# jw007123/hp-Adaptive-Signed-Distance-Field-Octree

Measured on AMD Instinct MI355X. Metric: Query() Mpts/sec at targetError=1e-5 (union3 field, 10M SplitMix64 pts per GPU, HBM-resident); Create() ms reported as create_ms, higher is better.
Workload: dtype f64

## Files before the change

### hp-adaptive-signed-distance-field-octree_amd/__init__.py

```python
import ctypes as C
import os

import numpy as np

_HERE = os.path.dirname(os.path.abspath(__file__))
_WHICH = os.environ.get("HPSDF_LIBRARY", "")
LIB_PATH = os.path.join(_HERE, "lib", "libhpsdf_%s.so" % _WHICH if _WHICH else "libhpsdf.so")
_LIB = None

OK = 0
ERR_INVALID_ARGUMENT = 1
ERR_NO_DEVICE = 2
ERR_HIP = 3
ERR_BAD_BLOCK = 4
ERR_UNSUPPORTED = 5
ERR_STATE = 6
ERR_OUT_OF_MEMORY = 7
ERR_OPEN_MESH = 8
ERR_BUILD_LIMIT = 9
ABI_VERSION = 4
PRIM_SPHERE, PRIM_BOX, PRIM_TORUS_Y, PRIM_PLANE = 0, 1, 2, 3
OP_UNION, OP_INTERSECT, OP_SUBTRACT = 0, 1, 2
JOB_HEADER_DOUBLES = 9
DEFAULT_JOBS_PER_ROUND = 1024
# ... 56 lines not shown
CALLBACK = C.CFUNCTYPE(C.c_double, C.POINTER(C.c_double), C.c_uint64, C.c_void_p)

_SIGNATURES = {
    "hpsdf_config_default": (C.c_int, [C.POINTER(PodConfig)]),
    "hpsdf_last_error": (C.c_char_p, []),
    "hpsdf_version": (C.c_char_p, []),
    "hpsdf_tables_get": (C.c_int, [C.c_void_p] * 7),
    "hpsdf_ctx_create": (C.c_int, [C.c_int, C.c_void_p, C.POINTER(C.c_void_p)]),
    "hpsdf_ctx_destroy": (C.c_int, [C.c_void_p]),
    "hpsdf_ctx_set_stream": (C.c_int, [C.c_void_p, C.c_void_p]),
    "hpsdf_ctx_synchronize": (C.c_int, [C.c_void_p]),
    "hpsdf_ctx_set_fast_fit": (C.c_int, [C.c_void_p, C.c_int]),
    "hpsdf_ctx_set_fit_mode": (C.c_int, [C.c_void_p, C.c_int]),
    "hpsdf_ctx_get_fit_mode": (C.c_int, [C.c_void_p, C.POINTER(C.c_int)]),
    "hpsdf_ctx_set_split_min_degree": (C.c_int, [C.c_void_p, C.c_int]),
    "hpsdf_ctx_set_block_allocator": (None, [C.c_void_p] * 4),
    "hpsdf_field_release_host_copies": (C.c_int, [C.c_void_p]),
    "hpsdf_set_mesh_face_rule": (None, [C.c_int]),
    "hpsdf_get_mesh_face_rule": (C.c_int, []),
    "hpsdf_set_reduction_order": (None, [C.c_int]),
    "hpsdf_get_reduction_order": (C.c_int, []),
    "hpsdf_ctx_stream": (C.c_void_p, [C.c_void_p]),
    "hpsdf_abi_version": (C.c_int, []),
    "hpsdf_ctx_set_reduction_order": (C.c_int, [C.c_void_p, C.c_int]),
    "hpsdf_ctx_get_reduction_order": (C.c_int, [C.c_void_p, C.POINTER(C.c_int)]),
    "hpsdf_ctx_set_mesh_face_rule": (C.c_int, [C.c_void_p, C.c_int]),
    "hpsdf_ctx_get_mesh_face_rule": (C.c_int, [C.c_void_p, C.POINTER(C.c_int)]),
    "hpsdf_ctx_set_build_limits": (C.c_int, [C.c_void_p, C.c_uint64, C.c_uint64]),
    "hpsdf_ctx_get_build_limits": (C.c_int, [C.c_void_p, C.POINTER(C.c_uint64), C.POINTER(C.c_uint64)]),
    "hpsdf_field_create_analytic": (C.c_int, [C.POINTER(Prim), C.c_int, C.POINTER(C.c_void_p)]),
# ... 106 lines not shown
                                                       C.POINTER(ContinuityStats)]),
    "hpsdf_continuity_matrix": (C.c_int, [C.c_void_p, C.c_size_t, C.c_uint64, C.POINTER(C.POINTER(C.c_uint64)),
                                          C.POINTER(C.POINTER(C.c_uint64)), C.POINTER(C.POINTER(C.c_double)),
                                          C.POINTER(ContinuityStats)]),
    "hpsdf_continuity_matrix_device": (C.c_int, [C.c_void_p, C.c_void_p, C.c_size_t, C.POINTER(C.POINTER(C.c_uint64)),
                                          C.POINTER(C.POINTER(C.c_uint64)), C.POINTER(C.POINTER(C.c_double)),
                                          C.POINTER(ContinuityStats)]),
    "hpsdf_continuity_last_stats": (C.c_int, [C.POINTER(ContinuityStats)]),
    "hpsdf_create": (C.c_int, [C.c_void_p, C.POINTER(PodConfig), C.c_void_p, C.c_uint64, C.POINTER(C.c_void_p),
                               C.POINTER(C.c_size_t), C.POINTER(BuildStats)]),
    "hpsdf_create_distributed": (C.c_int, [C.c_void_p, C.POINTER(PodConfig), C.c_void_p, C.c_uint64, C.c_int, C.c_int, C.c_void_p,
                                           C.c_void_p, C.POINTER(C.c_void_p), C.POINTER(C.c_size_t), C.POINTER(BuildStats)]),
    "hpsdf_fit_cells": (C.c_int, [C.c_void_p, C.POINTER(PodConfig), C.c_void_p, C.c_int, C.c_int, C.c_uint64, C.c_void_p, C.c_void_p]),
    "hpsdf_bench_fit": (C.c_int, [C.c_void_p, C.POINTER(PodConfig), C.c_void_p, C.c_int, C.c_int, C.c_uint64, C.c_int,
                                  C.POINTER(C.c_double)]),
}


def lib():
    global _LIB
    if _LIB is None:
        if not os.path.exists(LIB_PATH):
            raise ImportError("libhpsdf.so is not built (run __graft_entry__.build() or "
                              "python hp-adaptive-signed-distance-field-octree_amd/build.py); "
                              "there is no CPU fallback for the hot path")
        try:
            import torch
        except Exception:
            pass
        L = C.CDLL(LIB_PATH)
# ... 162 lines not shown

    def build_limits(self):
        a, b = C.c_uint64(), C.c_uint64()
        check(lib().hpsdf_ctx_get_build_limits(self.handle, C.byref(a), C.byref(b)))
        return a.value, b.value

    def set_fast_fit(self, on=True):
        check(lib().hpsdf_ctx_set_fast_fit(self.handle, 1 if on else 0))

    def set_fit_mode(self, mode):
        check(lib().hpsdf_ctx_set_fit_mode(self.handle, int(mode)))

    def set_split_min_degree(self, degree):
        check(lib().hpsdf_ctx_set_split_min_degree(self.handle, int(degree)))

    def fit_mode(self):
        m = C.c_int(0)
        check(lib().hpsdf_ctx_get_fit_mode(self.handle, C.byref(m)))
        return m.value

    def synchronize(self):
        check(lib().hpsdf_ctx_synchronize(self.handle))

    def close(self):
        if self.handle:
            lib().hpsdf_ctx_destroy(self.handle)
            self.handle = C.c_void_p()

    def __del__(self):
        try:
# ... 534 lines not shown

def bench_fit(ctx, config, field, degree, depth, n_cells, repeats=5):
    pod = config.to_pod()
    ms = C.c_double()
    check(lib().hpsdf_bench_fit(ctx.handle, C.byref(pod), field.handle, degree, depth, n_cells, repeats, C.byref(ms)))
    return ms.value


def fit_cells(ctx, config, field, degree, depth, n_cells):
    pod = config.to_pod()
    nc = int(NCOEF[degree])
    coeffs, errs = np.empty((n_cells, nc)), np.empty(n_cells)
    check(lib().hpsdf_fit_cells(ctx.handle, C.byref(pod), field.handle, degree, depth, n_cells, coeffs.ctypes.data_as(C.c_void_p),
                                errs.ctypes.data_as(C.c_void_p)))
    return coeffs, errs


class Octree:

    def __init__(self, device=0, stream=None, jobs_per_round=0):
        self._device, self._stream, self.K = device, stream, jobs_per_round
        self._ctx = None
        self._tree = None
        self.block = None
        self.config = None
        self.stats = None

    @property
    def ctx(self):
        if self._ctx is None:
# ... 419 lines not shown
```

### hp-adaptive-signed-distance-field-octree_amd/build.py

```python
import os
import shutil
import subprocess
import sys

HERE = os.path.dirname(os.path.abspath(__file__))
CSRC = os.path.join(HERE, "csrc")
LIBDIR = os.path.join(HERE, "lib")
LIB = os.path.join(LIBDIR, "libhpsdf.so")
HOOKS_LIB = os.path.join(LIBDIR, "libhpsdf_hooks.so")
HOOK_SOURCES = ["frontier.hip", "capi.cpp"]
INCLUDE = os.path.normpath(os.path.join(HERE, "..", "include"))

SOURCES = ["fit_mesh.hip", "fit_analytic.hip", "fit_samples.hip", "fit.hip", "kernels.hip", "mesh_field.hip", "frontier.hip", "fit_mfma.hip", "fit_low.hip", "mesh_build.hip", "cg.hip", "continuity_asm.hip", "surface.hip", "surface_sparse.hip", "query_gradient.hip", "query_hessian.hip", "project.hip", "cast_rays.hip", "query_bounds.hip", "integrate.hip", "tables.cpp", "builder.cpp", "mesh.cpp", "obj.cpp", "continuity.cpp", "host_query.cpp", "capi.cpp"]
HEADERS = sorted(f for f in os.listdir(CSRC) if f.endswith(".hpp"))
QUERY_SOURCES = ("kernels.hip",)
MESH_SOURCES = ("mesh_field.hip", "fit_mesh.hip")
SOURCE_GROUPS = {"query": QUERY_SOURCES, "mesh": MESH_SOURCES}
PUBLIC_HEADERS = ["hpsdf.h", "hpsdf_octree.hpp"]

FLAGS = ["-O3", "-std=c++17", "-fPIC", "-ffp-contract=off", "-fno-fast-math", "--offload-arch=gfx950",
         "-fvisibility=hidden", "-Wall", "-Wno-unused-function", "-I", INCLUDE]
FLAGS += os.environ.get("HPSDF_EXTRA_FLAGS", "").split()
FILE_FLAGS = {"fit_mfma.hip": ["-mllvm", "-amdgpu-mfma-vgpr-form=1"]}


def hipcc():
    for c in (os.environ.get("HIPCC"), "/opt/rocm/bin/hipcc", shutil.which("hipcc")):
        if c and os.path.exists(c):
            return c
    raise RuntimeError("hipcc not found: the HIP extension cannot be built (there is no CPU fallback)")


def stale():
    if not os.path.exists(LIB) or not os.path.exists(HOOKS_LIB):
        return True
    t = os.path.getmtime(LIB)
    deps = [os.path.join(CSRC, s) for s in SOURCES + HEADERS] + [os.path.join(INCLUDE, h) for h in PUBLIC_HEADERS]
    deps.append(os.path.abspath(__file__))
# ... 104 lines not shown
```

### hp-adaptive-signed-distance-field-octree_amd/csrc/capi.cpp

```cpp
#include <hip/hip_runtime_api.h>

#include <atomic>
#include <limits>
#include <cfloat>
#include <chrono>
#include <cmath>
#include <cstdio>
#include <cstdlib>
#include <cstring>
#include <memory>
#include <mutex>
#include <new>
#include <string>
#include <thread>
#include <vector>

#include "builder.hpp"
#include "continuity.hpp"
#include "frontier.hpp"
#include "block.hpp"
#include "host_call.hpp"
#include "integrate.hpp"
#include "launch.hpp"
#include "ray_cast.hpp"
#include "runtime.hpp"
#include "tree_bound.hpp"

using namespace hpsdf;

namespace hpsdf {

int loadObj(const char* path, std::vector<float>& verts, std::vector<uint64_t>& tris, std::string& err);

// ... 5 lines not shown
    g_lastError = msg;
    return code;
}
int hipFail(hipError_t e, const char* what) {
    g_lastError = std::string(what) + ": " + hipGetErrorString(e);
    (void)hipGetLastError();
    return (e == hipErrorNoDevice || e == hipErrorInvalidDevice || e == hipErrorInsufficientDriver) ? HPSDF_ERR_NO_DEVICE
                                                                                                 : HPSDF_ERR_HIP;
}

const hpsdf_field* innermost(const hpsdf_field* f) {
    while (f && f->kind == kHostTreeCsg) f = f->inner;
    return f;
}

static int envLeftAssoc() {
    const char* e = std::getenv("HPSDF_REDUCTION_ORDER");
    return e && (e[0] == 'l' || e[0] == 'L' || e[0] == '1');
}
static std::atomic<int> gLeftAssoc{envLeftAssoc()};
int reductionLeftAssoc(const hpsdf_ctx* ctx) { return ctx && ctx->reductionOrder >= 0 ? ctx->reductionOrder : gLeftAssoc.load(std::memory_order_relaxed); }
void setReductionLeftAssoc(int left) { gLeftAssoc.store(left != 0, std::memory_order_relaxed); }

static int envMeshFaceRule() {
    const char* e = std::getenv("HPSDF_MESH_FACE_RULE");
    return e && (e[0] == 'r' || e[0] == 'R' || e[0] == '1');
}
static std::atomic<int> gMeshFaceReference{envMeshFaceRule()};
int meshFaceRuleReference(const hpsdf_ctx* ctx) { return ctx && ctx->meshFaceRule >= 0 ? ctx->meshFaceRule : gMeshFaceReference.load(std::memory_order_relaxed); }
void setMeshFaceRuleReference(int on) { gMeshFaceReference.store(on != 0, std::memory_order_relaxed); }
// ... 61 lines not shown
            out->mesh.slabs = f->dSlabs;
            out->mesh.leafLog2 = f->leafLog2;
            {
                const char* pc = std::getenv("HPSDF_MESH_POOL_CAP");
                out->mesh.poolCap = pc ? (uint32_t)std::strtoul(pc, nullptr, 10) : 0xFFFFFFFFu;
            }
            out->mesh.nTris = f->nTris;
            out->mesh.nNodes = f->nBvhNodes;
            out->mesh.stats = f->dStats;
            out->mesh.faceTolOfSlack = meshFaceTolOfSlack(ctx);
            break;
        default:
            return fail(HPSDF_ERR_INVALID_ARGUMENT, "unknown field kind");
    }
    out->leftAssoc = reductionLeftAssoc(ctx);
    return HPSDF_OK;
}

}

namespace {
int treeOnContext(hpsdf_ctx* ctx, const hpsdf_tree* t, TreeDev* td = nullptr) {
    if (t->device != ctx->device) return fail(HPSDF_ERR_INVALID_ARGUMENT, "tree lives on another device");
    HPSDF_HIP(hipSetDevice(ctx->device));
    if (td) *td = t->dev, td->leftAssoc = reductionLeftAssoc(ctx);
    return HPSDF_OK;
}
}

extern "C" {
// ... 39 lines not shown
    *out = nullptr;
    int n = 0;
    hipError_t e = hipGetDeviceCount(&n);
    if (e != hipSuccess || n == 0)
        return fail(HPSDF_ERR_NO_DEVICE, std::string("no HIP device: ") + (e != hipSuccess ? hipGetErrorString(e) : "count = 0"));
    if (device < 0 || device >= n) return fail(HPSDF_ERR_INVALID_ARGUMENT, "device ordinal out of range");
    HPSDF_HIP(hipSetDevice(device));
    hpsdf_ctx* c = new hpsdf_ctx();
    c->device = device;
    c->splitMinDegree = fitSplitDefaultMinDegree();
    if (const char* fm = std::getenv("HPSDF_FIT_MODE")) {
        if (!std::strcmp(fm, "exact")) c->fitMode = HPSDF_FIT_EXACT;
        else if (!std::strcmp(fm, "fast")) c->fitMode = HPSDF_FIT_FAST;
        else if (!std::strcmp(fm, "split")) c->fitMode = HPSDF_FIT_SPLIT;
    }
    if (stream) {
        c->stream = (hipStream_t)stream;
    } else {
        hipError_t se = hipStreamCreateWithFlags(&c->stream, hipStreamNonBlocking);
        if (se != hipSuccess) {
            delete c;
            return hipFail(se, "hipStreamCreate");
        }
        c->ownsStream = true;
    }
    const Tables& T = tables();
    DeviceTables* h = new DeviceTables();
    std::memset(h, 0, sizeof(*h));
    std::memcpy(h->roots, T.roots, sizeof T.roots);
    std::memcpy(h->weights, T.weights, sizeof T.weights);
// ... 42 lines not shown
        c->ownsStream = false;
    }
    c->stream = (hipStream_t)stream;
    return HPSDF_OK;
}

int hpsdf_ctx_set_fit_mode(hpsdf_ctx* c, int mode) {
    if (!c) return fail(HPSDF_ERR_INVALID_ARGUMENT, "null context");
    if (mode != HPSDF_FIT_EXACT && mode != HPSDF_FIT_SPLIT && mode != HPSDF_FIT_FAST) return fail(HPSDF_ERR_INVALID_ARGUMENT, "unknown fit mode");
    c->fitMode = mode;
    return HPSDF_OK;
}
int hpsdf_ctx_get_fit_mode(hpsdf_ctx* c, int* mode) {
    if (!c || !mode) return fail(HPSDF_ERR_INVALID_ARGUMENT, "null argument");
    *mode = c->fitMode;
    return HPSDF_OK;
}
int hpsdf_ctx_set_build_limits(hpsdf_ctx* c, uint64_t max_nodes, uint64_t max_bytes) {
    if (!c) return fail(HPSDF_ERR_INVALID_ARGUMENT, "null context");
    c->limitNodes = max_nodes, c->limitBytes = max_bytes;
    return HPSDF_OK;
}
int hpsdf_ctx_get_build_limits(const hpsdf_ctx* c, uint64_t* max_nodes, uint64_t* max_bytes) {
    if (!c) return fail(HPSDF_ERR_INVALID_ARGUMENT, "null context");
    if (max_nodes) *max_nodes = c->limitNodes;
    if (max_bytes) *max_bytes = c->limitBytes;
    return HPSDF_OK;
}
int hpsdf_ctx_set_split_min_degree(hpsdf_ctx* c, int degree) {
    if (!c) return fail(HPSDF_ERR_INVALID_ARGUMENT, "null context");
// ... 1508 lines not shown
    if (!ctx) return fail(HPSDF_ERR_NO_DEVICE, "a device context is required");
    if (!block || !rowPtr || !col || !val) return fail(HPSDF_ERR_INVALID_ARGUMENT, "null argument");
    std::string err;
    const int rc = continuityMatrixDevice(ctx, block, size, rowPtr, col, val, stats, err);
    if (rc) return fail(rc, err);
    return HPSDF_OK;
    HPSDF_CATCH
}

int hpsdf_continuity_last_stats(hpsdf_continuity_stats* out) {
    if (!out) return fail(HPSDF_ERR_INVALID_ARGUMENT, "null out");
    *out = g_lastContinuity;
    return HPSDF_OK;
}

static int benchFit(hpsdf_ctx* ctx, const hpsdf_config* cfg, const hpsdf_field* field, int degree, int depth, uint64_t nCells, int repeats,
                    double* msPerLaunch, double* coeffsOut, double* errsOut);
int hpsdf_bench_fit(hpsdf_ctx* ctx, const hpsdf_config* cfg, const hpsdf_field* field, int degree, int depth,
                    uint64_t nCells, int repeats, double* msPerLaunch) {
    HPSDF_TRY
    if (!msPerLaunch) return fail(HPSDF_ERR_INVALID_ARGUMENT, "bad bench arguments");
    return benchFit(ctx, cfg, field, degree, depth, nCells, repeats, msPerLaunch, nullptr, nullptr);
    HPSDF_CATCH
}
int hpsdf_fit_cells(hpsdf_ctx* ctx, const hpsdf_config* cfg, const hpsdf_field* field, int degree, int depth, uint64_t nCells, double* coeffs,
                    double* errs) {
    HPSDF_TRY
    if (!coeffs || !errs) return fail(HPSDF_ERR_INVALID_ARGUMENT, "null argument");
    double ms = 0.0;
    return benchFit(ctx, cfg, field, degree, depth, nCells, 1, &ms, coeffs, errs);
// ... 113 lines not shown
```

### hp-adaptive-signed-distance-field-octree_amd/csrc/device_types.hpp

```cpp
#pragma once
#include <hip/hip_vector_types.h>

#include <cstdint>

#include "../../include/hpsdf.h"

namespace hpsdf {

struct DeviceTables {
    double roots[2080];
    double weights[2080];
    double nl[13][11];
    double rec[13][2];
    uint8_t bidx[456][4];
    uint32_t count[16];
};

struct NodeRec {
    uint32_t a, b;
};
constexpr uint32_t kInteriorTag = 0xFFFFFFFFu;

struct alignas(128) TopEntry {
    uint32_t a, b;
// ... 48 lines not shown
    const uint32_t* halfEdges;
    const BvhNode* bvh;
    const NodeSlab* slabs;
    uint32_t nTris, nNodes;
    uint32_t leafLog2;
    uint32_t poolCap;
    float faceTolOfSlack;
    unsigned long long* stats;
};

struct FieldDev {
    int32_t kind;
    int32_t nPrims;
    int32_t csgOp;
    int32_t leftAssoc;
    hpsdf_prim prims[HPSDF_MAX_PRIMS];
    const double* samples;
    MeshDev mesh;
    TreeDev oldTree;
};

struct RootMap {
    double bounds[3];
    double centre[3];
};

struct FitTask {
    float bmin[3], bmax[3];
    uint64_t outOff;
    uint64_t copyOff;
// ... 25 lines not shown
```

### hp-adaptive-signed-distance-field-octree_amd/csrc/field_eval.hpp

```cpp
#pragma once
#include <hip/hip_runtime.h>

#include "device_types.hpp"

namespace hpsdf {

template <bool LEFT>
__device__ __forceinline__ double sum3(double a, double b, double c) {
    if constexpr (LEFT) return (a + b) + c;
    else return a + (b + c);
}
template <bool LEFT>
__device__ __forceinline__ double prod3(double a, double b, double c) {
    if constexpr (LEFT) return (a * b) * c;
    else return a * (b * c);
}
__device__ __forceinline__ double sqrtExact(double x) {
    const uint32_t hi = (uint32_t)__double2hiint(x);
    const bool plain = hi - 0x10000000u < 0x7FF00000u - 0x10000000u;
    if (__builtin_amdgcn_ballot_w64(!plain) != 0ull) return sqrt(x);
    const double y = __builtin_amdgcn_rsq(x);
    double g = x * y, h = y * 0.5;
    const double r = __builtin_fma(-h, g, 0.5);
    g = __builtin_fma(g, r, g);
// ... 35 lines not shown

template <bool LEFT>
__device__ __forceinline__ double analyticEval(const FieldDev& f, double x, double y, double z) {
    double acc = primEval<LEFT>(f.prims[0], x, y, z);
    for (int i = 1; i < f.nPrims; ++i) {
        const double d = primEval<LEFT>(f.prims[i], x, y, z);
        switch (f.prims[i].op) {
            case HPSDF_OP_UNION: acc = fmin(acc, d); break;
            case HPSDF_OP_INTERSECT: acc = fmax(acc, d); break;
            default: acc = fmax(acc, -d); break;
        }
    }
    return acc;
}

}
```

### hp-adaptive-signed-distance-field-octree_amd/csrc/fit_kernels.hpp

```cpp
#pragma once
#include <hip/hip_runtime.h>

#include <cstdint>

#include "device_types.hpp"
#include "field_glue.hpp"
#include "launch.hpp"

namespace hpsdf {


constexpr int kFitPiece = 8;
#ifndef HPSDF_FIT_MIN_WAVES
#define HPSDF_FIT_MIN_WAVES 4
#endif

__device__ __forceinline__ double fitRowAny(double acc, double a1, const double* __restrict__ tk, double n2,
                                            const double* __restrict__ F, int nq) {
    int k = 0;
    for (; k + 4 <= nq; k += 4) {
        const double f0 = F[k], f1 = F[k + 1], f2 = F[k + 2], f3 = F[k + 3];
        const double t0 = tk[k], t1 = tk[k + 1], t2 = tk[k + 2], t3 = tk[k + 3];
        acc = acc + (a1 * t0 * n2) * f0;
        acc = acc + (a1 * t1 * n2) * f1;
        acc = acc + (a1 * t2 * n2) * f2;
        acc = acc + (a1 * t3 * n2) * f3;
    }
    for (; k < nq; ++k) acc = acc + (a1 * tk[k] * n2) * F[k];
    return acc;
}

template <int KIND, bool CSG, int DEG, int R, bool LEFT>
__device__ __forceinline__ void fitBlockBody(const FitBlock blk, const FitTask* __restrict__ tasks, double* __restrict__ arena,
                                             double* __restrict__ errs, double* __restrict__ mirror,
                                             const DeviceTables* __restrict__ T, const FieldDev& field, const RootMap& rm, double* lds) {
    static_assert(R == 1 || DEG > 0, "cell blocking needs a compile-time degree");
    __shared__ double sNl[13 * 11];
    __shared__ double sRec[26];
    __shared__ int32_t sMeshStack[kFitThreads / 64][kMeshStack];
    __shared__ unsigned char sPosI[KIND == kFieldMesh ? 64 : 4], sPosJK[KIND == kFieldMesh ? 64 : 4];
    const int tid = threadIdx.x;
    const int deg = DEG > 0 ? DEG : (int)blk.degree;
    const int nq = 4 * deg + 1, nq2 = nq * nq, G = blk.nTasks;
    const int rowStart = blk.rowStart, rowEnd = blk.rowEnd, nrows = rowEnd - rowStart;
    const int gl = nq * (nq - 1) / 2;
    const int planes = blk.planesPerChunk;
    const int depth = blk.depth;
    const bool split = blk.split != 0;

    double* sT = lds;
// ... 16 lines not shown
        }
    }
    for (int g = tid; g < G; g += kFitThreads) {
        const FitTask& tk = tasks[blk.firstTask + g];
        double sc[3];
        for (int a = 0; a < 3; ++a) {
            sc[a] = (double)(tk.bmax[a] - tk.bmin[a]) * 0.5;
            sC[8 * g + 3 + a] = (double)((tk.bmin[a] + tk.bmax[a]) / 2.0f);
            sC[8 * g + a] = sc[a];
        }
        sC[8 * g + 6] = prod3<LEFT>(sc[0], sc[1], sc[2]);
        sC[8 * g + 7] = __longlong_as_double((long long)tk.sampleOff);
    }
    __syncthreads();

    const bool wide = DEG == 0 && nrows > kFitThreads;
    const int slot = wide ? 0 : tid / nrows;
    const int g2 = slot * R;
    const int r0 = rowStart + (wide ? tid : tid % nrows);
    const int r1 = r0 + kFitThreads;
    const bool act0 = wide ? (r0 < rowEnd) : (tid < ((G + R - 1) / R) * nrows);
    const bool act1 = wide && r1 < rowEnd;
    int i0a = 0, i1a = 0, i2a = 0, i0b = 0, i1b = 0, i2b = 0;
    double n0a = 0, n1a = 0, n2a = 0, n0b = 0, n1b = 0, n2b = 0;
    if (act0) {
        i0a = T->bidx[r0][0], i1a = T->bidx[r0][1], i2a = T->bidx[r0][2];
        n0a = sNl[i0a * 11 + depth], n1a = sNl[i1a * 11 + depth], n2a = sNl[i2a * 11 + depth];
    }
    if (act1) {
        i0b = T->bidx[r1][0], i1b = T->bidx[r1][1], i2b = T->bidx[r1][2];
// ... 18 lines not shown
            if (tid < nq) {
                int rank = 0;
                for (int b = 0; b < nq; ++b) rank += sR[b] < sR[tid] ? 1 : 0;
                sPosJK[rank] = (unsigned char)tid;
            }
            if (tid >= 64 && tid < 64 + np) {
                const int a = tid - 64;
                int rank = 0;
                for (int b = 0; b < np; ++b) rank += sR[iBase + b] < sR[iBase + a] ? 1 : 0;
                sPosI[rank] = (unsigned char)a;
            }
            __syncthreads();
        }
        if constexpr (KIND != kFieldMesh) {
            const int cols = G * nq2;
            for (int c0 = 0; c0 < cols; c0 += kFitThreads) {
                const int cc = c0 + tid;
                const bool activeS = cc < cols;
                const int ccl = activeS ? cc : cols - 1;
                const int g = ccl / nq2, jk = ccl - g * nq2, j = jk / nq, k = jk - j * nq;
                const double* c = sC + 8 * g;
                const double uy = sR[j] * c[1] + c[4], uz = sR[k] * c[2] + c[5];
                const double wy = uy * rm.bounds[1] + rm.centre[1];
                const double wz = uz * rm.bounds[2] + rm.centre[2];
                const double wj = sW[j], wk = sW[k], c6 = c[6];
                const uint64_t sbase = (uint64_t)__double_as_longlong(c[7]) + (uint64_t)(j * nq + k);
                for (int il = 0; il < np; ++il) {
                    const int i = iBase + il;
                    const double ux = sR[i] * c[0] + c[3];
                    const double wx = ux * rm.bounds[0] + rm.centre[0];
                    const uint64_t sidx = sbase + (uint64_t)(i * nq2);
                    const double fv = activeS ? fieldEvalWorld<KIND, CSG, LEFT>(field, wx, wy, wz, sidx, sNl, sRec, meshHint) : 0.0;
                    if (activeS) {
                        sF[g * cellStride + il * nq2 + jk] = c6 * prod3<LEFT>(sW[i], wj, wk) * fv;
                        if (split) const_cast<double*>(field.samples)[sidx] = fv;
                    }
                }
            }
        } else {
            const int chunkSamples = np * nq2, total = G * chunkSamples;
            const float invChunk = 1.0f / (float)chunkSamples;
            for (int s0 = 0; s0 < total; s0 += kFitThreads) {
                const int s = s0 + tid;
                const bool activeS = s < total;
                const int sc = activeS ? s : total - 1;
                int g = (int)(((float)sc + 0.5f) * invChunk);
                int rem = sc - g * chunkSamples;
                if (rem < 0) {
                    --g;
                    rem += chunkSamples;
                } else if (rem >= chunkSamples) {
                    ++g;
                    rem -= chunkSamples;
// ... 116 lines not shown
            if (T->bidx[r][3] == deg) {
                const double c = sF[g * stashStride + (r - stashBase)];
                e = e + c * c;
            }
        errs[tasks[blk.firstTask + g].errSlot] = e;
    }
}

template <int KIND, bool CSG, bool LEFT>
__global__ __launch_bounds__(kFitThreads, HPSDF_FIT_MIN_WAVES) void fit_multi_kernel(const FitBlock* __restrict__ blocks,
                                                                const FitTask* __restrict__ tasks, double* __restrict__ arena,
                                                                double* __restrict__ errs, const DeviceTables* __restrict__ T,
                                                                FieldDev field, RootMap rm, const uint32_t* __restrict__ count,
                                                                uint32_t countValue) {
    extern __shared__ double lds[];
    const uint32_t n = count ? *count : countValue;
    if (blockIdx.x >= n) return;
    const FitBlock blk = blocks[n - 1u - blockIdx.x];
    switch (blk.degree) {
        case 2: fitBlockBody<KIND, CSG, 2, 1, LEFT>(blk, tasks, arena, errs, nullptr, T, field, rm, lds); break;
        case 3: fitBlockBody<KIND, CSG, 3, 1, LEFT>(blk, tasks, arena, errs, nullptr, T, field, rm, lds); break;
        case 4: fitBlockBody<KIND, CSG, 4, 1, LEFT>(blk, tasks, arena, errs, nullptr, T, field, rm, lds); break;
        case 5: fitBlockBody<KIND, CSG, 5, 1, LEFT>(blk, tasks, arena, errs, nullptr, T, field, rm, lds); break;
        case 6: fitBlockBody<KIND, CSG, 6, 1, LEFT>(blk, tasks, arena, errs, nullptr, T, field, rm, lds); break;
        case 7: fitBlockBody<KIND, CSG, 7, 1, LEFT>(blk, tasks, arena, errs, nullptr, T, field, rm, lds); break;
        case 8: fitBlockBody<KIND, CSG, 8, 1, LEFT>(blk, tasks, arena, errs, nullptr, T, field, rm, lds); break;
        default: fitBlockBody<KIND, CSG, 0, 1, LEFT>(blk, tasks, arena, errs, nullptr, T, field, rm, lds); break;
    }
}

template <int KIND, bool CSG, int DEG, int R, bool LEFT>
__global__ __launch_bounds__(kFitThreads, HPSDF_FIT_MIN_WAVES) void fit_kernel(const FitBlock* __restrict__ blocks,
                                                          const FitTask* __restrict__ tasks, double* __restrict__ arena,
                                                          double* __restrict__ errs, double* __restrict__ mirror,
                                                          const DeviceTables* __restrict__ T, FieldDev field, RootMap rm,
                                                          const uint32_t* __restrict__ range) {
    extern __shared__ double lds[];
    uint32_t b = blockIdx.x;
    if (range != nullptr) {
        if (b >= range[1]) return;
        b += range[0];
    }
    fitBlockBody<KIND, CSG, DEG, R, LEFT>(blocks[b], tasks, arena, errs, mirror, T, field, rm, lds);
}

template <int KIND, bool CSG, bool LEFT>
__global__ __launch_bounds__(256) void field_kernel(FieldDev f, const DeviceTables* __restrict__ T,
                                                    const double* __restrict__ xyz, size_t n, double* __restrict__ out) {
    __shared__ double sNl[13 * 11];
    __shared__ double sRec[26];
    stageQueryTables(T, sNl, sRec);
    __syncthreads();
    const size_t stride = (size_t)gridDim.x * blockDim.x;
    uint32_t hint = 0xFFFFFFFFu;
    for (size_t i = (size_t)blockIdx.x * blockDim.x + threadIdx.x; i < n; i += stride)
        out[i] = fieldEvalWorld<KIND, CSG, LEFT>(f, xyz[3 * i], xyz[3 * i + 1], xyz[3 * i + 2], i, sNl, sRec, hint);
}

// ... 84 lines not shown
```

### hp-adaptive-signed-distance-field-octree_amd/csrc/runtime.hpp

```cpp
#pragma once
#include <cstdlib>
#include <hip/hip_runtime_api.h>

#include <cstdint>
#include <atomic>
#include <exception>
#include <memory>
#include <mutex>
#include <new>
#include <string>
#include <vector>

#include "device_types.hpp"
#include "tables.hpp"

namespace hpsdf {

template <typename T>
struct Staged {
    T* dev = nullptr;
    T* host = nullptr;
    uint64_t cap = 0;
    hipError_t ensure(uint64_t n) {
        if (n <= cap) return hipSuccess;
// ... 46 lines not shown
}

namespace hpsdf {
struct IntegrateCell;
}

struct hpsdf_ctx {
    int device = 0;
    hipStream_t stream = nullptr;
    bool ownsStream = false;
    hpsdf::DeviceTables* dTables = nullptr;
    int fitMode = HPSDF_FIT_SPLIT;
    int splitMinDegree = 6;
    int reductionOrder = -1;
    int meshFaceRule = -1;
    uint64_t limitNodes = 0, limitBytes = 0;
    hpsdf::Workspace ws;
    std::shared_ptr<void> frontierScratch;
    std::shared_ptr<void> continuityScratch;
    char* hostDev = nullptr;
    size_t hostDevCap = 0;
    char* hostPin = nullptr;
    char* hostPinDev = nullptr;
    size_t hostPinCap = 0;
    std::mutex hostLock;
    std::mutex scratchLock;
    uint32_t* dDefer = nullptr;
    uint64_t deferCap = 0;
    uint32_t* dDeferCount = nullptr;
    void* (*blockAlloc)(size_t, void*) = nullptr;
// ... 160 lines not shown
```

### include/hpsdf.h

```cpp
#ifndef HPSDF_H
#define HPSDF_H

#include <stddef.h>
#include <stdint.h>

#ifdef __cplusplus
extern "C" {
#endif

#if defined(__GNUC__)
#define HPSDF_API __attribute__((visibility("default")))
#else
#define HPSDF_API
#endif

typedef enum hpsdf_status {
    HPSDF_OK = 0,
    HPSDF_ERR_INVALID_ARGUMENT = 1,
    HPSDF_ERR_NO_DEVICE = 2,
    HPSDF_ERR_HIP = 3,
    HPSDF_ERR_BAD_BLOCK = 4,
    HPSDF_ERR_UNSUPPORTED = 5,
    HPSDF_ERR_STATE = 6,
    HPSDF_ERR_OUT_OF_MEMORY = 7,
// ... 43 lines not shown
HPSDF_API const char* hpsdf_version(void);

HPSDF_API int hpsdf_tables_get(double* roots, double* weights, double* normalised_lengths, double* recurrence,
                               uint64_t* coeff_count, uint64_t* basis_index, uint64_t* sum_to_n);

typedef struct hpsdf_ctx hpsdf_ctx;
HPSDF_API int hpsdf_ctx_create(int device, void* stream, hpsdf_ctx** out);
HPSDF_API int hpsdf_ctx_destroy(hpsdf_ctx* ctx);
HPSDF_API int hpsdf_ctx_set_stream(hpsdf_ctx* ctx, void* stream);
HPSDF_API int hpsdf_ctx_synchronize(hpsdf_ctx* ctx);
enum { HPSDF_FIT_EXACT = 0, HPSDF_FIT_SPLIT = 1, HPSDF_FIT_FAST = 2 };
HPSDF_API int hpsdf_ctx_set_fit_mode(hpsdf_ctx* ctx, int mode);
HPSDF_API int hpsdf_ctx_get_fit_mode(hpsdf_ctx* ctx, int* mode);
HPSDF_API int hpsdf_ctx_set_split_min_degree(hpsdf_ctx* ctx, int degree);
HPSDF_API int hpsdf_ctx_set_fast_fit(hpsdf_ctx* ctx, int on);
HPSDF_API void hpsdf_set_reduction_order(int left_assoc);
HPSDF_API int hpsdf_get_reduction_order(void);
HPSDF_API int hpsdf_ctx_set_reduction_order(hpsdf_ctx* ctx, int left_assoc);
HPSDF_API int hpsdf_ctx_get_reduction_order(const hpsdf_ctx* ctx, int* left_assoc);
HPSDF_API int hpsdf_ctx_set_build_limits(hpsdf_ctx* ctx, uint64_t max_nodes, uint64_t max_bytes);
HPSDF_API int hpsdf_ctx_get_build_limits(const hpsdf_ctx* ctx, uint64_t* max_nodes, uint64_t* max_bytes);
HPSDF_API void* hpsdf_ctx_stream(hpsdf_ctx* ctx);

enum { HPSDF_PRIM_SPHERE = 0, HPSDF_PRIM_BOX = 1, HPSDF_PRIM_TORUS_Y = 2, HPSDF_PRIM_PLANE = 3 };
enum { HPSDF_OP_UNION = 0, HPSDF_OP_INTERSECT = 1, HPSDF_OP_SUBTRACT = 2 };
#define HPSDF_MAX_PRIMS 16
typedef struct hpsdf_prim {
    int32_t kind;
    int32_t op;
    double p[8];
// ... 230 lines not shown
typedef void (*hpsdf_block_release_fn)(void* block, void* user);
HPSDF_API void hpsdf_ctx_set_block_allocator(hpsdf_ctx* ctx, hpsdf_block_alloc_fn alloc, hpsdf_block_release_fn release, void* user);

HPSDF_API int hpsdf_create(hpsdf_ctx* ctx, const hpsdf_config* cfg, const hpsdf_field* field,
                           uint64_t max_jobs_per_round, void** block, size_t* size, hpsdf_build_stats* stats);

typedef int (*hpsdf_allgather_fn)(void* user, void* d_buf, size_t bytes_per_rank, void* stream);
HPSDF_API int hpsdf_create_distributed(hpsdf_ctx* ctx, const hpsdf_config* cfg, const hpsdf_field* field,
                                       uint64_t max_jobs_per_round, int rank, int world, hpsdf_allgather_fn gather,
                                       void* user, void** block, size_t* size, hpsdf_build_stats* stats);

HPSDF_API int hpsdf_bench_fit(hpsdf_ctx* ctx, const hpsdf_config* cfg, const hpsdf_field* field, int degree,
                              int depth, uint64_t n_cells, int repeats, double* ms_per_launch);
HPSDF_API int hpsdf_fit_cells(hpsdf_ctx* ctx, const hpsdf_config* cfg, const hpsdf_field* field, int degree, int depth,
                              uint64_t n_cells, double* coeffs, double* errs);

#ifdef __cplusplus
}
#endif
#endif
```

Before: 94960.

## Cull analytic CSG primitives per fit cell using conservative distance intervals

Before sampling, each fit block computes a conservative interval for every analytic primitive's signed distance over each cell, using a Lipschitz bound around the cell centre. It folds these intervals to find which primitives can affect the union/intersect result. Sample evaluation then skips primitives that no lane in the wave needs, and uses a single-primitive fast path when only one remains. The goal is to cut field evaluations during Create() fitting, at the cost of an extra prepass, shared-memory use and added wave-level control flow; the Query throughput metric is not directly targeted.

```diff
diff --git a/hp-adaptive-signed-distance-field-octree_amd/__init__.py b/hp-adaptive-signed-distance-field-octree_amd/__init__.py
--- a/hp-adaptive-signed-distance-field-octree_amd/__init__.py
+++ b/hp-adaptive-signed-distance-field-octree_amd/__init__.py
@@ -94,6 +94,8 @@
     "hpsdf_ctx_set_fit_mode": (C.c_int, [C.c_void_p, C.c_int]),
     "hpsdf_ctx_get_fit_mode": (C.c_int, [C.c_void_p, C.POINTER(C.c_int)]),
     "hpsdf_ctx_set_split_min_degree": (C.c_int, [C.c_void_p, C.c_int]),
+    "hpsdf_ctx_set_fit_cull": (C.c_int, [C.c_void_p, C.c_int]),
+    "hpsdf_ctx_get_fit_cull": (C.c_int, [C.c_void_p, C.POINTER(C.c_int)]),
     "hpsdf_ctx_set_block_allocator": (None, [C.c_void_p] * 4),
     "hpsdf_field_release_host_copies": (C.c_int, [C.c_void_p]),
     "hpsdf_set_mesh_face_rule": (None, [C.c_int]),
@@ -230,6 +232,7 @@
     "hpsdf_fit_cells": (C.c_int, [C.c_void_p, C.POINTER(PodConfig), C.c_void_p, C.c_int, C.c_int, C.c_uint64, C.c_void_p, C.c_void_p]),
     "hpsdf_bench_fit": (C.c_int, [C.c_void_p, C.POINTER(PodConfig), C.c_void_p, C.c_int, C.c_int, C.c_uint64, C.c_int,
                                   C.POINTER(C.c_double)]),
+    "hpsdf_fit_cull_masks": (C.c_int, [C.POINTER(PodConfig), C.c_void_p, C.c_int, C.c_uint64, C.c_void_p, C.c_void_p]),
 }
 
 
@@ -422,6 +425,14 @@
     def set_split_min_degree(self, degree):
         check(lib().hpsdf_ctx_set_split_min_degree(self.handle, int(degree)))
 
+    def set_fit_cull(self, on):
+        check(lib().hpsdf_ctx_set_fit_cull(self.handle, -1 if on is None else (1 if on else 0)))
+
+    def fit_cull(self):
+        v = C.c_int(0)
+        check(lib().hpsdf_ctx_get_fit_cull(self.handle, C.byref(v)))
+        return v.value
+
     def fit_mode(self):
         m = C.c_int(0)
         check(lib().hpsdf_ctx_get_fit_mode(self.handle, C.byref(m)))
@@ -986,6 +997,14 @@
     check(lib().hpsdf_fit_cells(ctx.handle, C.byref(pod), field.handle, degree, depth, n_cells, coeffs.ctypes.data_as(C.c_void_p),
                                 errs.ctypes.data_as(C.c_void_p)))
     return coeffs, errs
+
+
+def fit_cull_masks(config, field, depth, n_cells):
+    pod = config.to_pod()
+    first, mask = np.empty(n_cells, np.uint32), np.empty(n_cells, np.uint32)
+    check(lib().hpsdf_fit_cull_masks(C.byref(pod), field.handle, depth, n_cells, first.ctypes.data_as(C.c_void_p),
+                                     mask.ctypes.data_as(C.c_void_p)))
+    return first, mask
 
 
 class Octree:
diff --git a/hp-adaptive-signed-distance-field-octree_amd/build.py b/hp-adaptive-signed-distance-field-octree_amd/build.py
--- a/hp-adaptive-signed-distance-field-octree_amd/build.py
+++ b/hp-adaptive-signed-distance-field-octree_amd/build.py
@@ -21,7 +21,8 @@
 FLAGS = ["-O3", "-std=c++17", "-fPIC", "-ffp-contract=off", "-fno-fast-math", "--offload-arch=gfx950",
          "-fvisibility=hidden", "-Wall", "-Wno-unused-function", "-I", INCLUDE]
 FLAGS += os.environ.get("HPSDF_EXTRA_FLAGS", "").split()
-FILE_FLAGS = {"fit_mfma.hip": ["-mllvm", "-amdgpu-mfma-vgpr-form=1"]}
+FILE_FLAGS = {"fit_mfma.hip": ["-mllvm", "-amdgpu-mfma-vgpr-form=1"],
+              "fit_analytic.hip": ["-mllvm", "-instcombine-max-copied-from-constant-users=4096"]}
 
 
 def hipcc():
diff --git a/hp-adaptive-signed-distance-field-octree_amd/csrc/capi.cpp b/hp-adaptive-signed-distance-field-octree_amd/csrc/capi.cpp
--- a/hp-adaptive-signed-distance-field-octree_amd/csrc/capi.cpp
+++ b/hp-adaptive-signed-distance-field-octree_amd/csrc/capi.cpp
@@ -17,6 +17,7 @@
 
 #include "builder.hpp"
 #include "continuity.hpp"
+#include "fit_cull.hpp"
 #include "frontier.hpp"
 #include "block.hpp"
 #include "host_call.hpp"
@@ -52,6 +53,10 @@
     return f;
 }
 
+static int envFitCull() {
+    const char* e = std::getenv("HPSDF_FIT_CULL");
+    return !(e && e[0] == '0');
+}
 static int envLeftAssoc() {
     const char* e = std::getenv("HPSDF_REDUCTION_ORDER");
     return e && (e[0] == 'l' || e[0] == 'L' || e[0] == '1');
@@ -143,6 +148,7 @@
             return fail(HPSDF_ERR_INVALID_ARGUMENT, "unknown field kind");
     }
     out->leftAssoc = reductionLeftAssoc(ctx);
+    out->fitCull = (ctx && ctx->fitCull && out->kind == kFieldAnalytic && out->csgOp < 0 && out->nPrims > 1) ? 1 : 0;
     return HPSDF_OK;
 }
 
@@ -212,6 +218,7 @@
         else if (!std::strcmp(fm, "fast")) c->fitMode = HPSDF_FIT_FAST;
         else if (!std::strcmp(fm, "split")) c->fitMode = HPSDF_FIT_SPLIT;
     }
+    c->fitCull = envFitCull();
     if (stream) {
         c->stream = (hipStream_t)stream;
     } else {
@@ -284,6 +291,17 @@
 int hpsdf_ctx_get_fit_mode(hpsdf_ctx* c, int* mode) {
     if (!c || !mode) return fail(HPSDF_ERR_INVALID_ARGUMENT, "null argument");
     *mode = c->fitMode;
+    return HPSDF_OK;
+}
+int hpsdf_ctx_set_fit_cull(hpsdf_ctx* c, int on) {
+    if (!c) return fail(HPSDF_ERR_INVALID_ARGUMENT, "null context");
+    if (on < -1 || on > 1) return fail(HPSDF_ERR_INVALID_ARGUMENT, "fit cull: -1 (the default: on unless HPSDF_FIT_CULL=0), 0 or 1");
+    c->fitCull = on < 0 ? envFitCull() : on;
+    return HPSDF_OK;
+}
+int hpsdf_ctx_get_fit_cull(const hpsdf_ctx* c, int* on) {
+    if (!c || !on) return fail(HPSDF_ERR_INVALID_ARGUMENT, "null argument");
+    *on = c->fitCull;
     return HPSDF_OK;
 }
 int hpsdf_ctx_set_build_limits(hpsdf_ctx* c, uint64_t max_nodes, uint64_t max_bytes) {
@@ -1822,6 +1840,73 @@
     return HPSDF_OK;
 }
 
+namespace {
+double hostSum3(double a, double b, double c, int left) { return left ? (a + b) + c : a + (b + c); }
+double hostPrimEval(const hpsdf_prim& pr, double x, double y, double z, int left) {
+    const double* p = pr.p;
+    switch (pr.kind) {
+        case HPSDF_PRIM_SPHERE: {
+            const double dx = x - p[0], dy = y - p[1], dz = z - p[2];
+            return std::sqrt(hostSum3(dx * dx, dy * dy, dz * dz, left)) - p[3];
+        }
+        case HPSDF_PRIM_BOX: {
+            const double qx = std::fabs(x - p[0]) - p[3], qy = std::fabs(y - p[1]) - p[4], qz = std::fabs(z - p[2]) - p[5];
+            const double ox = std::fmax(qx, 0.0), oy = std::fmax(qy, 0.0), oz = std::fmax(qz, 0.0);
+            const double outside = std::sqrt(hostSum3(ox * ox, oy * oy, oz * oz, left));
+            const double inside = std::fmin(std::fmax(qx, std::fmax(qy, qz)), 0.0);
+            return outside + inside;
+        }
+        case HPSDF_PRIM_TORUS_Y: {
+            const double dx = x - p[0], dy = y - p[1], dz = z - p[2];
+            const double l = std::sqrt(dx * dx + dz * dz) - p[3];
+            return std::sqrt(l * l + dy * dy) - p[4];
+        }
+        case HPSDF_PRIM_PLANE: return (p[0] * x + (p[1] * y + p[2] * z)) + p[3];
+        default: return 0.0;
+    }
+}
+}
+
+int hpsdf_fit_cull_masks(const hpsdf_config* cfg, const hpsdf_field* field, int depth, uint64_t nCells, uint32_t* firstOut, uint32_t* maskOut) {
+    HPSDF_TRY
+    if (!cfg || !field || !firstOut || !maskOut || depth < 0 || depth > kMaxDepth) return fail(HPSDF_ERR_INVALID_ARGUMENT, "bad fit_cull_masks arguments");
+    const hpsdf_field* in = innermost(field);
+    if (!in || in->kind != kHostAnalytic) return fail(HPSDF_ERR_UNSUPPORTED, "fit_cull_masks needs an analytic field");
+    const int nP = (int)in->prims.size();
+    const bool wrapped = field->kind == kHostTreeCsg;
+    const int left = reductionLeftAssoc(nullptr);
+    double rb[3], rc[3];
+    for (int a = 0; a < 3; ++a) {
+        rb[a] = (double)(cfg->root_max[a] - cfg->root_min[a]);
+        rc[a] = (double)((cfg->root_min[a] + cfg->root_max[a]) / 2.0f);
+    }
+    const uint64_t side = 1ull << depth;
+    const float h = 1.0f / (float)side;
+    double iv[2 * HPSDF_MAX_PRIMS];
+    for (uint64_t n = 0; n < nCells; ++n) {
+        const uint64_t c = n % (side * side * side);
+        const uint64_t ix[3] = {c % side, (c / side) % side, c / (side * side)};
+        double ce[3], he[3];
+        for (int a = 0; a < 3; ++a) {
+            const float bmin = -0.5f + (float)ix[a] * h, bmax = bmin + h;
+            ce[a] = (double)((bmin + bmax) / 2.0f) * rb[a] + rc[a];
+            he[a] = (double)(bmax - bmin) * 0.5 * std::fabs(rb[a]);
+        }
+        int first = 0;
+        uint32_t mask = nP >= 32 ? 0xFFFFFFFFu : (1u << nP) - 1u;
+        if (!wrapped) {
+            const double r = cullRadius(he[0], he[1], he[2]), cm = cullCentreMax(ce[0], ce[1], ce[2]);
+            for (int i = 0; i < nP; ++i)
+                cullInterval(in->prims[i], hostPrimEval(in->prims[i], ce[0], ce[1], ce[2], left), r, cm, i > 0 && cullNegates(in->prims[i].op),
+                             iv[2 * i], iv[2 * i + 1]);
+            cullFold(in->prims.data(), nP, iv, first, mask);
+        }
+        firstOut[n] = (uint32_t)first, maskOut[n] = mask;
+    }
+    return HPSDF_OK;
+    HPSDF_CATCH
+}
+
 static int benchFit(hpsdf_ctx* ctx, const hpsdf_config* cfg, const hpsdf_field* field, int degree, int depth, uint64_t nCells, int repeats,
                     double* msPerLaunch, double* coeffsOut, double* errsOut);
 int hpsdf_bench_fit(hpsdf_ctx* ctx, const hpsdf_config* cfg, const hpsdf_field* field, int degree, int depth,
diff --git a/hp-adaptive-signed-distance-field-octree_amd/csrc/device_types.hpp b/hp-adaptive-signed-distance-field-octree_amd/csrc/device_types.hpp
--- a/hp-adaptive-signed-distance-field-octree_amd/csrc/device_types.hpp
+++ b/hp-adaptive-signed-distance-field-octree_amd/csrc/device_types.hpp
@@ -86,6 +86,8 @@
     int32_t nPrims;
     int32_t csgOp;
     int32_t leftAssoc;
+    int32_t fitCull;
+    int32_t pad0;
     hpsdf_prim prims[HPSDF_MAX_PRIMS];
     const double* samples;
     MeshDev mesh;
diff --git a/hp-adaptive-signed-distance-field-octree_amd/csrc/field_eval.hpp b/hp-adaptive-signed-distance-field-octree_amd/csrc/field_eval.hpp
--- a/hp-adaptive-signed-distance-field-octree_amd/csrc/field_eval.hpp
+++ b/hp-adaptive-signed-distance-field-octree_amd/csrc/field_eval.hpp
@@ -73,4 +73,26 @@
     return acc;
 }
 
+template <bool LEFT>
+__device__ __forceinline__ double analyticEvalCulled(const FieldDev& f, int first, uint32_t mask, uint32_t need, double x, double y,
+                                                     double z) {
+    double acc = 0.0;
+    for (int i = 0; i < f.nPrims; ++i) {
+        if (((need >> i) & 1u) == 0u) continue;
+        const int op = i > 0 ? f.prims[i].op : HPSDF_OP_UNION;
+        double v = primEval<LEFT>(f.prims[i], x, y, z);
+        if (op != HPSDF_OP_UNION && op != HPSDF_OP_INTERSECT) v = -v;
+        const double folded = op == HPSDF_OP_UNION ? fmin(acc, v) : fmax(acc, v);
+        acc = i == first ? v : ((mask >> i) & 1u) != 0u ? folded : acc;
+    }
+    return acc;
 }
+
+__device__ __forceinline__ uint32_t cullWaveNeed(int nPrims, uint32_t mask) {
+    uint32_t need = 0u;
+    for (int i = 0; i < nPrims; ++i)
+        if (__builtin_amdgcn_ballot_w64(((mask >> i) & 1u) != 0u) != 0ull) need |= 1u << i;
+    return need;
+}
+
+}
diff --git a/hp-adaptive-signed-distance-field-octree_amd/csrc/fit_cull.hpp b/hp-adaptive-signed-distance-field-octree_amd/csrc/fit_cull.hpp
--- /dev/null
+++ b/hp-adaptive-signed-distance-field-octree_amd/csrc/fit_cull.hpp
@@ -0,0 +1,76 @@
+#pragma once
+#include <hip/hip_runtime_api.h>
+
+#include <cfloat>
+#include <cmath>
+#include <cstdint>
+
+#include "../../include/hpsdf.h"
+
+namespace hpsdf {
+
+constexpr double kCullEps = 1.0 / 1073741824.0;
+
+__host__ __device__ __forceinline__ bool cullFinite(double v) { return fabs(v) <= DBL_MAX; }
+
+__host__ __device__ __forceinline__ double cullRadius(double hx, double hy, double hz) {
+    return sqrt(hx * hx + (hy * hy + hz * hz)) * (1.0 + kCullEps);
+}
+
+__host__ __device__ __forceinline__ double cullCentreMax(double cx, double cy, double cz) {
+    double m = fabs(cx);
+    if (fabs(cy) > m) m = fabs(cy);
+    if (fabs(cz) > m) m = fabs(cz);
+    return m;
+}
+
+__host__ __device__ __forceinline__ void cullInterval(const hpsdf_prim& pr, double dc, double r, double centreMax, bool negate, double& lo,
+                                             double& hi) {
+    const double* p = pr.p;
+    double L = 1.0;
+    if (pr.kind == HPSDF_PRIM_PLANE) L = sqrt(p[0] * p[0] + (p[1] * p[1] + p[2] * p[2]));
+    double pm = 0.0;
+    for (int j = 0; j < 8; ++j)
+        if (fabs(p[j]) > pm) pm = fabs(p[j]);
+    const double Lr = L * r;
+    const double s = kCullEps * (fabs(dc) + Lr + pm + centreMax + 1.0);
+    const double a = dc - Lr - s, b = dc + Lr + s;
+    lo = negate ? -b : a;
+    hi = negate ? -a : b;
+}
+
+__host__ __device__ __forceinline__ bool cullNegates(int op) { return op != HPSDF_OP_UNION && op != HPSDF_OP_INTERSECT; }
+
+__host__ __device__ __forceinline__ void cullFold(const hpsdf_prim* prims, int n, const double* iv, int& first, uint32_t& mask) {
+    const uint32_t all = n >= 32 ? 0xFFFFFFFFu : (1u << n) - 1u;
+    first = 0, mask = all;
+    if (n <= 1) return;
+    for (int i = 0; i < n; ++i)
+        if (!cullFinite(iv[2 * i]) || !cullFinite(iv[2 * i + 1])) return;
+    double alo = iv[0], ahi = iv[1];
+    int f = 0;
+    uint32_t m = 1u;
+    for (int i = 1; i < n; ++i) {
+        const double lo = iv[2 * i], hi = iv[2 * i + 1];
+        if (prims[i].op == HPSDF_OP_UNION) {
+            if (lo > ahi) {
+            } else if (hi < alo) {
+                f = i, m = 1u << i;
+            } else {
+                m |= 1u << i;
+            }
+            alo = lo < alo ? lo : alo, ahi = hi < ahi ? hi : ahi;
+        } else {
+            if (hi < alo) {
+            } else if (lo > ahi) {
+                f = i, m = 1u << i;
+            } else {
+                m |= 1u << i;
+            }
+            alo = lo > alo ? lo : alo, ahi = hi > ahi ? hi : ahi;
+        }
+    }
+    first = f, mask = m;
+}
+
+}
diff --git a/hp-adaptive-signed-distance-field-octree_amd/csrc/fit_kernels.hpp b/hp-adaptive-signed-distance-field-octree_amd/csrc/fit_kernels.hpp
--- a/hp-adaptive-signed-distance-field-octree_amd/csrc/fit_kernels.hpp
+++ b/hp-adaptive-signed-distance-field-octree_amd/csrc/fit_kernels.hpp
@@ -2,15 +2,18 @@
 #include <hip/hip_runtime.h>
 
 #include <cstdint>
+#include <type_traits>
 
 #include "device_types.hpp"
 #include "field_glue.hpp"
+#include "fit_cull.hpp"
 #include "launch.hpp"
 
 namespace hpsdf {
 
 
 constexpr int kFitPiece = 8;
+constexpr int kFitCullCells = 64;
 #ifndef HPSDF_FIT_MIN_WAVES
 #define HPSDF_FIT_MIN_WAVES 4
 #endif
@@ -33,7 +36,7 @@
 template <int KIND, bool CSG, int DEG, int R, bool LEFT>
 __device__ __forceinline__ void fitBlockBody(const FitBlock blk, const FitTask* __restrict__ tasks, double* __restrict__ arena,
                                              double* __restrict__ errs, double* __restrict__ mirror,
-                                             const DeviceTables* __restrict__ T, const FieldDev& field, const RootMap& rm, double* lds) {
+                                             const DeviceTables* __restrict__ T, const FieldDev& field, const RootMap& rm, double* lds, uint32_t* sCull) {
     static_assert(R == 1 || DEG > 0, "cell blocking needs a compile-time degree");
     __shared__ double sNl[13 * 11];
     __shared__ double sRec[26];
@@ -80,6 +83,34 @@
     }
     __syncthreads();
 
+    bool cull = false;
+    if constexpr (KIND == kFieldAnalytic && !CSG) {
+        const int nP = field.nPrims;
+        cull = field.fitCull != 0 && nP > 1 && deg >= 2 && G <= kFitCullCells;
+        if (cull) {
+            for (int i = __builtin_amdgcn_readfirstlane(tid >> 6); i < nP; i += kFitThreads / 64) {
+                const hpsdf_prim& pr = field.prims[i];
+                for (int g = tid & 63; g < G; g += 64) {
+                    const double* c = sC + 8 * g;
+                    const double cx = c[3] * rm.bounds[0] + rm.centre[0];
+                    const double cy = c[4] * rm.bounds[1] + rm.centre[1];
+                    const double cz = c[5] * rm.bounds[2] + rm.centre[2];
+                    const double r = cullRadius(c[0] * fabs(rm.bounds[0]), c[1] * fabs(rm.bounds[1]), c[2] * fabs(rm.bounds[2]));
+                    double* iv = sF + 2 * (g * nP + i);
+                    cullInterval(pr, primEval<LEFT>(pr, cx, cy, cz), r, cullCentreMax(cx, cy, cz), i > 0 && cullNegates(pr.op), iv[0], iv[1]);
+                }
+            }
+            __syncthreads();
+            for (int g = tid; g < G; g += kFitThreads) {
+                int first;
+                uint32_t mask;
+                cullFold(field.prims, nP, sF + 2 * g * nP, first, mask);
+                sCull[g] = (uint32_t)first << 16 | mask;
+            }
+            __syncthreads();
+        }
+    }
+
     const bool wide = DEG == 0 && nrows > kFitThreads;
     const int slot = wide ? 0 : tid / nrows;
     const int g2 = slot * R;
@@ -128,29 +159,58 @@
         }
         if constexpr (KIND != kFieldMesh) {
             const int cols = G * nq2;
-            for (int c0 = 0; c0 < cols; c0 += kFitThreads) {
-                const int cc = c0 + tid;
-                const bool activeS = cc < cols;
-                const int ccl = activeS ? cc : cols - 1;
-                const int g = ccl / nq2, jk = ccl - g * nq2, j = jk / nq, k = jk - j * nq;
-                const double* c = sC + 8 * g;
-                const double uy = sR[j] * c[1] + c[4], uz = sR[k] * c[2] + c[5];
-                const double wy = uy * rm.bounds[1] + rm.centre[1];
-                const double wz = uz * rm.bounds[2] + rm.centre[2];
-                const double wj = sW[j], wk = sW[k], c6 = c[6];
-                const uint64_t sbase = (uint64_t)__double_as_longlong(c[7]) + (uint64_t)(j * nq + k);
-                for (int il = 0; il < np; ++il) {
-                    const int i = iBase + il;
-                    const double ux = sR[i] * c[0] + c[3];
-                    const double wx = ux * rm.bounds[0] + rm.centre[0];
-                    const uint64_t sidx = sbase + (uint64_t)(i * nq2);
-                    const double fv = activeS ? fieldEvalWorld<KIND, CSG, LEFT>(field, wx, wy, wz, sidx, sNl, sRec, meshHint) : 0.0;
-                    if (activeS) {
-                        sF[g * cellStride + il * nq2 + jk] = c6 * prod3<LEFT>(sW[i], wj, wk) * fv;
-                        if (split) const_cast<double*>(field.samples)[sidx] = fv;
+            auto columns = [&](auto culled) {
+                constexpr bool CULL = decltype(culled)::value;
+                for (int c0 = 0; c0 < cols; c0 += kFitThreads) {
+                    const int cc = c0 + tid;
+                    const bool activeS = cc < cols;
+                    const int ccl = activeS ? cc : cols - 1;
+                    const int g = ccl / nq2, jk = ccl - g * nq2, j = jk / nq, k = jk - j * nq;
+                    const double* c = sC + 8 * g;
+                    const double uy = sR[j] * c[1] + c[4], uz = sR[k] * c[2] + c[5];
+                    const double wy = uy * rm.bounds[1] + rm.centre[1];
+                    const double wz = uz * rm.bounds[2] + rm.centre[2];
+                    const double wj = sW[j], wk = sW[k], c6 = c[6];
+                    const uint64_t sbase = (uint64_t)__double_as_longlong(c[7]) + (uint64_t)(j * nq + k);
+                    int cullFirst = 0;
+                    uint32_t cullMask = 0u, cullNeed = 0u;
+                    if constexpr (CULL) {
+                        const uint32_t fm = sCull[g];
+                        cullFirst = (int)(fm >> 16), cullMask = fm & 0xFFFFu;
+                        cullNeed = cullWaveNeed(field.nPrims, cullMask);
                     }
-                }
-            }
+                    auto planesOf = [&](auto eval) {
+                        for (int il = 0; il < np; ++il) {
+                            const int i = iBase + il;
+                            const double ux = sR[i] * c[0] + c[3];
+                            const double wx = ux * rm.bounds[0] + rm.centre[0];
+                            const uint64_t sidx = sbase + (uint64_t)(i * nq2);
+                            const double fv = activeS ? eval(wx, sidx) : 0.0;
+                            if (activeS) {
+                                sF[g * cellStride + il * nq2 + jk] = c6 * prod3<LEFT>(sW[i], wj, wk) * fv;
+                                if (split) const_cast<double*>(field.samples)[sidx] = fv;
+                            }
+                        }
+                    };
+                    if constexpr (CULL) {
+                        if ((cullNeed & (cullNeed - 1u)) == 0u) {
+                            const int only = __builtin_ctz(cullNeed);
+                            const hpsdf_prim& pr = field.prims[only];
+                            const bool neg = only > 0 && cullNegates(pr.op);
+                            planesOf([&](double wx, uint64_t) {
+                                const double d = primEval<LEFT>(pr, wx, wy, wz);
+                                return neg ? -d : d;
+                            });
+                        } else {
+                            planesOf([&](double wx, uint64_t) { return analyticEvalCulled<LEFT>(field, cullFirst, cullMask, cullNeed, wx, wy, wz); });
+                        }
+                    } else {
+                        planesOf([&](double wx, uint64_t sidx) { return fieldEvalWorld<KIND, CSG, LEFT>(field, wx, wy, wz, sidx, sNl, sRec, meshHint); });
+                    }
+                }
+            };
+            if (KIND == kFieldAnalytic && !CSG && cull) columns(std::true_type{});
+            else columns(std::false_type{});
         } else {
             const int chunkSamples = np * nq2, total = G * chunkSamples;
             const float invChunk = 1.0f / (float)chunkSamples;
@@ -297,18 +357,19 @@
                                                                 FieldDev field, RootMap rm, const uint32_t* __restrict__ count,
                                                                 uint32_t countValue) {
     extern __shared__ double lds[];
+    __shared__ uint32_t sCull[kFitCullCells];
     const uint32_t n = count ? *count : countValue;
     if (blockIdx.x >= n) return;
     const FitBlock blk = blocks[n - 1u - blockIdx.x];
     switch (blk.degree) {
-        case 2: fitBlockBody<KIND, CSG, 2, 1, LEFT>(blk, tasks, arena, errs, nullptr, T, field, rm, lds); break;
-        case 3: fitBlockBody<KIND, CSG, 3, 1, LEFT>(blk, tasks, arena, errs, nullptr, T, field, rm, lds); break;
-        case 4: fitBlockBody<KIND, CSG, 4, 1, LEFT>(blk, tasks, arena, errs, nullptr, T, field, rm, lds); break;
-        case 5: fitBlockBody<KIND, CSG, 5, 1, LEFT>(blk, tasks, arena, errs, nullptr, T, field, rm, lds); break;
-        case 6: fitBlockBody<KIND, CSG, 6, 1, LEFT>(blk, tasks, arena, errs, nullptr, T, field, rm, lds); break;
-        case 7: fitBlockBody<KIND, CSG, 7, 1, LEFT>(blk, tasks, arena, errs, nullptr, T, field, rm, lds); break;
-        case 8: fitBlockBody<KIND, CSG, 8, 1, LEFT>(blk, tasks, arena, errs, nullptr, T, field, rm, lds); break;
-        default: fitBlockBody<KIND, CSG, 0, 1, LEFT>(blk, tasks, arena, errs, nullptr, T, field, rm, lds); break;
+        case 2: fitBlockBody<KIND, CSG, 2, 1, LEFT>(blk, tasks, arena, errs, nullptr, T, field, rm, lds, sCull); break;
+        case 3: fitBlockBody<KIND, CSG, 3, 1, LEFT>(blk, tasks, arena, errs, nullptr, T, field, rm, lds, sCull); break;
+        case 4: fitBlockBody<KIND, CSG, 4, 1, LEFT>(blk, tasks, arena, errs, nullptr, T, field, rm, lds, sCull); break;
+        case 5: fitBlockBody<KIND, CSG, 5, 1, LEFT>(blk, tasks, arena, errs, nullptr, T, field, rm, lds, sCull); break;
+        case 6: fitBlockBody<KIND, CSG, 6, 1, LEFT>(blk, tasks, arena, errs, nullptr, T, field, rm, lds, sCull); break;
+        case 7: fitBlockBody<KIND, CSG, 7, 1, LEFT>(blk, tasks, arena, errs, nullptr, T, field, rm, lds, sCull); break;
+        case 8: fitBlockBody<KIND, CSG, 8, 1, LEFT>(blk, tasks, arena, errs, nullptr, T, field, rm, lds, sCull); break;
+        default: fitBlockBody<KIND, CSG, 0, 1, LEFT>(blk, tasks, arena, errs, nullptr, T, field, rm, lds, sCull); break;
     }
 }
 
@@ -319,12 +380,13 @@
                                                           const DeviceTables* __restrict__ T, FieldDev field, RootMap rm,
                                                           const uint32_t* __restrict__ range) {
     extern __shared__ double lds[];
+    __shared__ uint32_t sCull[kFitCullCells];
     uint32_t b = blockIdx.x;
     if (range != nullptr) {
         if (b >= range[1]) return;
         b += range[0];
     }
-    fitBlockBody<KIND, CSG, DEG, R, LEFT>(blocks[b], tasks, arena, errs, mirror, T, field, rm, lds);
+    fitBlockBody<KIND, CSG, DEG, R, LEFT>(blocks[b], tasks, arena, errs, mirror, T, field, rm, lds, sCull);
 }
 
 template <int KIND, bool CSG, bool LEFT>
diff --git a/hp-adaptive-signed-distance-field-octree_amd/csrc/runtime.hpp b/hp-adaptive-signed-distance-field-octree_amd/csrc/runtime.hpp
--- a/hp-adaptive-signed-distance-field-octree_amd/csrc/runtime.hpp
+++ b/hp-adaptive-signed-distance-field-octree_amd/csrc/runtime.hpp
@@ -84,6 +84,7 @@
     int splitMinDegree = 6;
     int reductionOrder = -1;
     int meshFaceRule = -1;
+    int fitCull = 1;
     uint64_t limitNodes = 0, limitBytes = 0;
     hpsdf::Workspace ws;
     std::shared_ptr<void> frontierScratch;
diff --git a/include/hpsdf.h b/include/hpsdf.h
--- a/include/hpsdf.h
+++ b/include/hpsdf.h
@@ -81,6 +81,8 @@
 HPSDF_API int hpsdf_ctx_get_fit_mode(hpsdf_ctx* ctx, int* mode);
 HPSDF_API int hpsdf_ctx_set_split_min_degree(hpsdf_ctx* ctx, int degree);
 HPSDF_API int hpsdf_ctx_set_fast_fit(hpsdf_ctx* ctx, int on);
+HPSDF_API int hpsdf_ctx_set_fit_cull(hpsdf_ctx* ctx, int on);
+HPSDF_API int hpsdf_ctx_get_fit_cull(const hpsdf_ctx* ctx, int* on);
 HPSDF_API void hpsdf_set_reduction_order(int left_assoc);
 HPSDF_API int hpsdf_get_reduction_order(void);
 HPSDF_API int hpsdf_ctx_set_reduction_order(hpsdf_ctx* ctx, int left_assoc);
@@ -341,6 +343,8 @@
                               int depth, uint64_t n_cells, int repeats, double* ms_per_launch);
 HPSDF_API int hpsdf_fit_cells(hpsdf_ctx* ctx, const hpsdf_config* cfg, const hpsdf_field* field, int degree, int depth,
                               uint64_t n_cells, double* coeffs, double* errs);
+HPSDF_API int hpsdf_fit_cull_masks(const hpsdf_config* cfg, const hpsdf_field* field, int depth, uint64_t n_cells,
+                                   uint32_t* first_out, uint32_t* mask_out);
 
 #ifdef __cplusplus
 }
```

Result: no change. 94670 (-0.3%).
